# EduFdez/rgbd360

Hardware: AMD Instinct MI355X
Metric: Gauss-Newton iters/sec on 2048x1024 spherical pair; SE(3) err vs CPU ref (higher is better)
Workload: dtype f32; 1 GPU; configs[1]: single 2048x1024 synthetic sphere pair per GPU, PHOTO_CONSISTENCY RegisterPhotoICP, level-0 forced Gauss-Newton iterations (one launch each: solve of the previous pass + fused warp/residual/Jacobian pass); width=2048, height=1024, method=PHOTO_CONSISTENCY, n_pyr=4, pairs_per_gpu=1, parallelism=1 GPU

## Files before the change

rgbd360_amd/csrc/photo_icp_kernels.h:

```cpp
#pragma once
#include <hip/hip_runtime.h>
#include <stddef.h>
#include <stdint.h>

#include "device_math.h"
#include "gn_math.h"
#include "libm_f32.h"
#include "partial_row.h"

namespace r360 {

constexpr float  kInvalidPoint = -10000.f;
constexpr int    kEvalThreads = 1024;

struct F3 {
    float a, b, c;
};

struct LevelDev {
    int rows, cols, n;
    float half_nRows;
    float angle_res_inv;
    float pi_k;
    const float4* src;
// ... 530 lines not shown
    ESTAMP(4);
    if (threadIdx.x == 0 && (b == 0 || b == nb - 1)) {
        double* o = partials + (size_t)(nb + (b == 0 ? 0 : 1)) * kNumPartials;
        for (int k = 0; k < 5; ++k) o[k] = (double)es[k];
        o[5] = (double)es0;
        }
    if (threadIdx.x == 0) {
        double* pb = partials + (size_t)(nb + 8) * kNumPartials + 2 * b;
        pb[0] = (double)es0;
        pb[1] = (double)(es0 + es[4]);
    }
    if (threadIdx.x == 0 && b == 0) {
        {
            unsigned long long* cnt = reinterpret_cast<unsigned long long*>(partials + (size_t)(nb + 2) * kNumPartials);
            const unsigned long long slot = atomicAdd(cnt, 1ull) % 60;
            double* h = partials + (size_t)(nb + 3) * kNumPartials + 2 * slot;
            h[0] = (double)es0;
            h[1] = (double)(es0 + es[4]);
        }
    }
#endif
}

template <int METHOD, bool HG, int THREADS = kEvalThreads, int SRC = 0>
__device__ __forceinline__ void eval_block(const GNState* __restrict__ st, const float4* __restrict__ src0, const int n_px,
                                           const int chunk, const int level, const int nb_arg, double* __restrict__ partials,
                                           const LevelDev& lv, const EvalConsts& ec) {
    unsigned long long es[6] = {0, 0, 0, 0, 0, 0};
#ifdef RGBD360_EVAL_STAMPS
    const unsigned long long es0 = __builtin_amdgcn_s_memrealtime();
#else
    const unsigned long long es0 = 0;
#endif
    const int nb = nb_arg;
    const int b = blockIdx.x;
    const int cb = ((nb & 7) == 0) ? (b & 7) * (nb >> 3) + (b >> 3) : b;
    const int base = cb * chunk;
    const int end = min(base + chunk, n_px);
    EvalBufs bufs;
    bufs.src = make_rsrc(src0, (unsigned)n_px * 16u);
    bufs.trgP = make_rsrc(lv.trgP, (unsigned)lv.n * 12u);
    bufs.trgD = make_rsrc(lv.trgD, (unsigned)lv.n * 12u);
    bufs.row_bytes = (unsigned)lv.cols * 12u;
    const int i = base + (int)threadIdx.x;
    static_assert(THREADS == 1024 || THREADS == 512, "eval_block: 1024-lane layout, played by 1024 or 512 threads");
    SrcCursor cur = {0, 0, 0, 0};
    SrcForm<SRC>::cursor_init(cur, lv, i, THREADS);
    const typename SrcForm<SRC>::T sA = SrcForm<SRC>::load(lv, src0, n_px, base, (unsigned)threadIdx.x << 4, cur);
    const typename SrcForm<SRC>::T sB = SrcForm<SRC>::load(lv, src0, n_px, base + THREADS, (unsigned)threadIdx.x << 4, cur);
    const int2 gate = *reinterpret_cast<const int2*>(&st->done);
    const PoseRT T = load_pose(st->cand);
    const WarpConsts wc = make_warp_consts(T, lv);
    ESTAMP(0);
    PixW wA;
    warp_stage<METHOD, true, SRC>(sA, i < end, T, wc, lv, bufs, wA);
    asm volatile("" ::: "memory");
    if (gate.x | (gate.y != level)) return;
    ESTAMP(1);
    eval_span<METHOD, HG, THREADS, SRC>(T, wc, lv, ec, bufs, src0, n_px, base, end, b, nb, wA, sB, cur, partials, es, es0);
}

template <int METHOD, bool HG, int SRC = 0>
__global__ __launch_bounds__(kEvalThreads) void k_eval(const GNState* __restrict__ st, const float4* __restrict__ src0, int n_px,
                                                        int chunk, int level, int nb_arg, double* __restrict__ partials,
                                                        LevelDev lv, EvalConsts ec) {
    eval_block<METHOD, HG, kEvalThreads, SRC>(st, src0, n_px, chunk, level, nb_arg, partials, lv, ec);
}

constexpr int kEvalThreadsBatch = 512;
template <int METHOD, bool HG, int SRC = 0>
__global__ __launch_bounds__(kEvalThreadsBatch) void k_eval_b(const GNState* __restrict__ states, const float4* __restrict__ src0, int n_px,
                                                          int chunk, int level, int nb_arg, double* __restrict__ partials,
                                                          int partials_stride, LevelDev lv, EvalConsts ec) {
    const int slot = blockIdx.y;
    lv.trgP += (size_t)slot * (size_t)n_px;
    lv.trgD += (size_t)slot * (size_t)n_px;
    if (SRC == 2) lv.src2 += (size_t)slot * (size_t)n_px;
    eval_block<METHOD, HG, kEvalThreadsBatch, SRC>(states + slot, SRC == 0 ? src0 + (size_t)slot * (size_t)n_px : src0, n_px, chunk, level, nb_arg,
                                                   partials + (size_t)slot * (size_t)partials_stride, lv, ec);
}

struct PairTable {
    int trg[32], src[32];
};
template <int METHOD, bool HG, int SRC = 0>
__global__ __launch_bounds__(kEvalThreadsBatch) void k_eval_p(const GNState* __restrict__ states, const float4* __restrict__ src0, int n_px,
                                                          int chunk, int level, int nb_arg, double* __restrict__ partials,
                                                          int partials_stride, LevelDev lv, EvalConsts ec, PairTable pt) {
    const int slot = blockIdx.y;
    const size_t to = (size_t)pt.trg[slot] * (size_t)n_px, so = (size_t)pt.src[slot] * (size_t)n_px;
    lv.trgP += to;
    lv.trgD += to;
    if (SRC == 2) lv.src2 += so;
    eval_block<METHOD, HG, kEvalThreadsBatch, SRC>(states + slot, SRC == 0 ? src0 + so : src0, n_px, chunk, level, nb_arg,
                                                   partials + (size_t)slot * (size_t)partials_stride, lv, ec);
}

struct Pose16 {
    float v[16];
};
__device__ __forceinline__ void level_init_one(GNState* st, const Pose16& pose, int use_pose, int reset_all, int level);
struct FsInit {
    Pose16 pose;
    int on;
};
__global__ void k_level_init(GNState* st, Pose16 pose, int use_pose, int reset_all, int level) {
    if (threadIdx.x != 0 || blockIdx.x != 0) return;
    level_init_one(st, pose, use_pose, reset_all, level);
}
__global__ void k_level_init_b(GNState* states, Pose16 pose, int use_pose, int reset_all, int level, unsigned long long live_mask) {
    if (threadIdx.x != 0) return;
    GNState* st = states + blockIdx.x;
    if (!((live_mask >> blockIdx.x) & 1ull)) {
        st->done = 1;
        st->level_active = -1;
        st->status = 0;
        return;
    }
    level_init_one(st, pose, use_pose, reset_all, level);
}
__global__ void k_level_init_p(GNState* states, const Pose16* __restrict__ poses, int use_pose, int reset_all, int level,
                               unsigned long long live_mask) {
    if (threadIdx.x != 0) return;
    GNState* st = states + blockIdx.x;
    if (!((live_mask >> blockIdx.x) & 1ull)) {
        st->done = 1;
        st->level_active = -1;
        st->status = 0;
        return;
    }
    level_init_one(st, poses[blockIdx.x], use_pose, reset_all, level);
}
__device__ __forceinline__ void level_init_one(GNState* st, const Pose16& pose, int use_pose, int reset_all, int level) {
    if (reset_all) {
        for (int k = 0; k < 36; ++k) st->H[k] = st->Hused[k] = 0.f;
        for (int k = 0; k < 6; ++k) st->g[k] = st->gused[k] = 0.f;
        for (int k = 0; k < 8; ++k) st->iters[k] = 0;
        st->status = 0;
        st->n_evals = 0;
        st->acc_e2p = st->acc_e2d = 0.0;
        st->acc_np = st->acc_nd = st->acc_nvis = st->used_nvis = st->used_npix = 0;
    } else {
        if (st->status != 0 || !st->done || st->level_active != level + 1) return;
    }
    st->level_active = level;
    st->pend_nb = 0;
    if (use_pose)
        for (int k = 0; k < 16; ++k) st->pose[k] = pose.v[k];
    for (int k = 0; k < 16; ++k) st->cand[k] = st->pose[k];
    for (int k = 0; k < 6; ++k) st->update[k] = 1.f;
    st->lambda = 1.0;
    st->it = 0;
    st->first = 1;
    st->done = 0;
    st->error = st->new_error = st->diff_error = 0.0;
}

__device__ __forceinline__ float bcast(float v, int lane_uniform) {
    return __builtin_bit_cast(float, __builtin_amdgcn_readlane(__builtin_bit_cast(int, v), lane_uniform));
}

__device__ __forceinline__ bool lu_inverse6_lanes(const float* M , int lane, float x[6]) {
    float a[6];
#pragma unroll
    for (int r = 0; r < 6; ++r) a[r] = lane < 6 ? M[lane * 6 + r] : ((lane - 6) == r ? 1.f : 0.f);
    bool ok = true;
    float rk[6];
#pragma unroll
    for (int k = 0; k < 6; ++k) {
        float ck[6];
#pragma unroll
        for (int r = k; r < 6; ++r) ck[r] = bcast(a[r], k);
        int piv = k;
        unsigned best = __float_as_uint(ck[k]) & 0x7fffffffu;
#pragma unroll
        for (int r = k + 1; r < 6; ++r) {
            const unsigned v = __float_as_uint(ck[r]) & 0x7fffffffu;
            if (v > best) {
                best = v;
                piv = r;
            }
        }
        if (best == 0u) ok = false;
        const int pv = __builtin_amdgcn_readfirstlane(piv);
        if (pv != k) {
#pragma unroll
            for (int r = k + 1; r < 6; ++r)
                if (pv == r) {
                    asm volatile("v_swap_b32 %0, %1" : "+v"(a[k]), "+v"(a[r]));
                    const float t = ck[k]; ck[k] = ck[r]; ck[r] = t;
                }
        }
        rk[k] = rcp_rn(ck[k]);
#pragma unroll
        for (int r = k + 1; r < 6; ++r) {
            const float l = ck[r] * rk[k];
            if (lane > k) a[r] -= l * a[k];
        }
    }
#pragma unroll
    for (int r = 5; r >= 0; --r) {
        float sacc = a[r];
#pragma unroll
        for (int c = r + 1; c < 6; ++c) sacc -= bcast(a[r], c) * x[c];
        x[r] = sacc * rk[r];
    }
    return ok;
}

__device__ __forceinline__ int qr_rank6_lanes(const float* M , int lane) {
    const int col = lane < 6 ? lane : 5;
    float a[6];
#pragma unroll
    for (int r = 0; r < 6; ++r) a[r] = M[col * 6 + r];
    float sq = 0.f;
#pragma unroll
    for (int r = 0; r < 6; ++r) sq += a[r] * a[r];
    float maxColSq = 0.f;
#pragma unroll
    for (int c = 0; c < 6; ++c) {
        const float v = bcast(sq, c);
        maxColSq = v > maxColSq ? v : maxColSq;
    }
    const float threshold_helper = maxColSq * (gn::kEpsF * gn::kEpsF) / 6.f;
    float pivots[6] = {0.f, 0.f, 0.f, 0.f, 0.f, 0.f};
    float maxpivot = 0.f;
    int nonzero = 6;
    bool stopped = false;
#pragma unroll
    for (int k = 0; k < 6; ++k) {
        float sk = 0.f;
#pragma unroll
        for (int r = k; r < 6; ++r) sk += a[r] * a[r];
        int best = k;
        float bestSq = -1.f;
#pragma unroll
        for (int c = k; c < 6; ++c) {
            const float v = bcast(sk, c);
            if (v > bestSq) {
                bestSq = v;
                best = c;
            }
        }
        if (!stopped && bestSq < threshold_helper * (float)(6 - k)) {
            nonzero = k;
            stopped = true;
        }
        if (!stopped) {
            if (best != k) {
#pragma unroll
                for (int r = 0; r < 6; ++r) {
                    const float from_best = bcast(a[r], best), from_k = bcast(a[r], k);
                    a[r] = (lane == k) ? from_best : ((lane == best) ? from_k : a[r]);
                }
            }
            float ck[6];
#pragma unroll
            for (int r = 0; r < 6; ++r) ck[r] = bcast(a[r], k);
            float tailSq = 0.f;
#pragma unroll
            for (int r = k + 1; r < 6; ++r) tailSq += ck[r] * ck[r];
            const float c0 = ck[k];
            float beta, tau;
            float v[6] = {0.f, 0.f, 0.f, 0.f, 0.f, 0.f};
            if (tailSq == 0.f) {
                tau = 0.f;
                beta = c0;
            } else {
                beta = sqrtf(c0 * c0 + tailSq);
                if (c0 >= 0.f) beta = -beta;
                const float den = c0 - beta;
#pragma unroll
                for (int r = k + 1; r < 6; ++r) v[r] = ck[r] / den;
                tau = (beta - c0) / beta;
            }
            v[k] = 1.f;
            float dot = 0.f;
#pragma unroll
            for (int r = k; r < 6; ++r) dot += v[r] * a[r];
            dot *= tau;
            if (lane > k) {
#pragma unroll
                for (int r = k; r < 6; ++r) a[r] -= dot * v[r];
            }
            pivots[k] = beta;
            const float ab = fabsf(beta);
            maxpivot = ab > maxpivot ? ab : maxpivot;
        }
    }
    const float thr = maxpivot * (gn::kEpsF * 6.f);
    int rank = 0;
#pragma unroll
    for (int k = 0; k < 6; ++k) rank += (k < nonzero && fabsf(pivots[k]) > thr) ? 1 : 0;
    return rank;
}

constexpr int kSolveThreads = 1024;
struct SolveShared {
    GNState sst;
    double red[kSolveThreads / 64][kNumPartials];
    float shH[36], shM[36], shInv[36], shE[16], shCand[16], shUpd[6];
    int shGo, shRank, shLuOk;
    unsigned long long stamp0, stamp[8];
};
#ifdef RGBD360_SOLVE_STAMPS
#define SOLVE_STAMP_T(i, t) if (threadIdx.x == (t)) sh.stamp[i] = __builtin_amdgcn_s_memrealtime() - sh.stamp0
#else
#define SOLVE_STAMP_T(i, t)
#endif
#define SOLVE_STAMP(i) SOLVE_STAMP_T(i, 0)

__device__ __forceinline__ void reduce_rows_to_lds(SolveShared& sh, double s) {
    const double pair = add_other_half_d(s);
    if ((threadIdx.x & 63) < kNumPartials) sh.red[threadIdx.x >> 6][threadIdx.x & 31] = pair;
}
__device__ __forceinline__ float solve_totals(SolveShared& sh) {
    constexpr int Q = kSolveThreads / 64;
    const int tid = threadIdx.x;
    if (tid < kNumPartials) {
        double t = 0.0;
#pragma unroll
        for (int k = 0; k < Q; ++k) t += sh.red[k][tid];
        sh.sst.tot[tid] = t;
    }
    const float lam_spec = (float)(sh.sst.first ? sh.sst.lambda : sh.sst.lambda / 5.0);
    __syncthreads();
    SOLVE_STAMP_T(1, 0);
    return lam_spec;
}

__device__ __forceinline__ int solve_rank_wave(SolveShared& sh, const float lam_spec) {
    const int lane = threadIdx.x & 63;
    const double* tot = sh.sst.tot;
    float hval = 0.f;
    if (lane < 36) {
        const int r = lane / 6, c = lane - 6 * r;
        const int aa = r < c ? r : c, bb = r < c ? c : r;
        hval = (float)tot[P_H + (aa * (13 - aa)) / 2 + (bb - aa)];
        sh.shM[lane] = (lane % 7 == 0) ? hval + lam_spec * hval : hval;
    }
    const int rk = __builtin_amdgcn_readfirstlane(qr_rank6_lanes(sh.shM, lane));
    if (lane == 0) sh.shRank = rk;
    return rk;
}

__device__ __forceinline__ void solve_waves(SolveShared& sh, const SolveCfg& cfg, const float lam_spec, const bool rank_now) {
    const int tid = threadIdx.x, lane = tid & 63, wave = tid >> 6;
    GNState* st = &sh.sst;
    const double* tot = sh.sst.tot;
    if (cfg.mode == 0 && wave == 2 && rank_now) {
        solve_rank_wave(sh, lam_spec);
        SOLVE_STAMP_T(7, 128);
    }
    if (cfg.mode == 0 && wave == 1) {
        float hval = 0.f;
        if (lane < 36) {
            const int r = lane / 6, c = lane - 6 * r;
            const int aa = r < c ? r : c, bb = r < c ? c : r;
            hval = (float)tot[P_H + (aa * (13 - aa)) / 2 + (bb - aa)];
        }
        {
            if (lane < 36) sh.shH[lane] = hval;
            float x[6] = {0.f, 0.f, 0.f, 0.f, 0.f, 0.f};
            const bool ok = lu_inverse6_lanes(sh.shH, lane, x);
            if (lane >= 6 && lane < 12) {
#pragma unroll
                for (int r = 0; r < 6; ++r) sh.shInv[(lane - 6) * 6 + r] = x[r];
            }
            if (lane == 0) sh.shLuOk = ok ? 1 : 0;
            SOLVE_STAMP_T(5, 64);
            float upd = 0.f;
            if (lane < 6) {
#pragma unroll
                for (int c = 0; c < 6; ++c) upd += (-sh.shInv[c * 6 + lane]) * (float)tot[P_G + c];
                sh.shUpd[lane] = upd;
            }
            const double ux = (double)bcast(upd, 0), uy = (double)bcast(upd, 1), uz = (double)bcast(upd, 2);
            const double wx = (double)bcast(upd, 3), wy = (double)bcast(upd, 4), wz = (double)bcast(upd, 5);
            const double theta_sq = wx * wx + wy * wy + wz * wz;
            double ca = 0.0, cb = 0.0;
            const bool rot = theta_sq >= (128 * 2.220446049250313e-16) * (128 * 2.220446049250313e-16);
            if (rot) {
                if (theta_sq < 0.25) gn::sinc_cosc_sq(theta_sq, ca, cb);
                else gn::sinc_cosc(sqrt(theta_sq), ca, cb);
            }
            if (lane < 16) {
                const int i = lane & 3, j = lane >> 2;
                double e = (i == j) ? 1.0 : 0.0;
                if (i < 3 && j < 3) {
                    if (rot) {
                        const double wi = i == 0 ? wx : (i == 1 ? wy : wz), wj = j == 0 ? wx : (j == 1 ? wy : wz);
                        const int kk = 3 - i - j;
                        const double wk = kk == 0 ? wx : (kk == 1 ? wy : wz);
                        double Wij, W2ij;
                        if (i == j) {
                            Wij = 0.0;
                            const double first = i == 2 ? wy : wz, second = i == 0 ? wy : wx;
                            W2ij = (0.0 - first * first) - second * second;
                        } else {
                            Wij = ((j - i + 3) % 3 == 1) ? -wk : wk;
                            W2ij = wi * wj;
                        }
                        e += ca * Wij + cb * W2ij;
                    }
                } else if (j == 3 && i < 3) {
                    e = i == 0 ? ux : (i == 1 ? uy : uz);
                }
                sh.shE[lane] = (float)e;
            }
            if (lane < 16) {
                const int c = lane >> 2, r = lane & 3;
                const float* P = sh.sst.cand;
                sh.shCand[lane] = ((sh.shE[0 * 4 + r] * P[c * 4 + 0] + sh.shE[1 * 4 + r] * P[c * 4 + 1]) + sh.shE[2 * 4 + r] * P[c * 4 + 2]) +
                               sh.shE[3 * 4 + r] * P[c * 4 + 3];
            }
            SOLVE_STAMP_T(6, 64);
        }
    }
    if (wave == 0) {
        float hval = 0.f;
        if (lane < 36) {
            const int r = lane / 6, c = lane - 6 * r;
            const int aa = r < c ? r : c, bb = r < c ? c : r;
            hval = (float)tot[P_H + (aa * (13 - aa)) / 2 + (bb - aa)];
        } else if (lane < 42) {
            hval = (float)tot[P_G + lane - 36];
        }
        int take = 0, go = 0;
        if (lane == 0) {
            st->n_evals += 1;
            const double err2 = tot[P_E2P] + tot[P_E2D];
            const double nvalid = tot[P_NP] + tot[P_ND];
            const double new_error = cfg.occ == 0 ? sqrt(err2 / nvalid)
                                                  : sqrt(tot[P_E2P] / tot[P_NP]) + sqrt(tot[P_E2D] / tot[P_ND]);
            st->new_error = new_error;
            if (cfg.mode == 1) {
                take = 1;
            } else {
                bool stop = false;
                if (st->first) {
                    st->first = 0;
                    if (nvalid == 0.0 || new_error != new_error) {
                        st->status = 2;
                        st->done = 1;
                        stop = true;
                    } else {
                        st->error = new_error;
                        st->diff_error = new_error;
                        take = 1;
                    }
                } else {
                    const double diff = st->error - new_error;
                    st->diff_error = diff;
                    if (cfg.forced || diff > cfg.tol_residual) {
                        st->lambda = st->lambda / 5.0;
                        st->error = new_error;
                        st->it += 1;
                        st->iters[cfg.level & 7] = st->it;
                        take = 2;
                    }
                }
                if (take) {
                    st->acc_e2p = tot[P_E2P];
                    st->acc_e2d = tot[P_E2D];
                    st->acc_np = (long long)tot[P_NP];
                    st->acc_nd = (long long)tot[P_ND];
                    st->acc_nvis = (long long)tot[P_NVIS];
                }
                if (!stop) {
                    float un = 0.f;
                    for (int i = 0; i < 6; ++i) un += st->update[i] * st->update[i];
                    un = sqrtf(un);
                    go = cfg.forced || (st->it < cfg.max_iters && (double)un > cfg.tol_update && st->diff_error > cfg.tol_residual);
                    if (!go) st->done = 1;
                }
                if (go) {
                    st->used_nvis = st->acc_nvis;
                    st->used_npix = cfg.n_pixels;
                }
            }
            sh.shGo = go;
        }
        take = __builtin_amdgcn_readfirstlane(take);
        go = __builtin_amdgcn_readfirstlane(go);
        if (take == 2 && lane < 16) st->pose[lane] = st->cand[lane];
        if (take) {
            if (lane < 36) st->H[lane] = hval;
            else if (lane < 42) st->g[lane - 36] = hval;
        }
        if (go) {
            if (lane < 36) {
                st->Hused[lane] = hval;
            } else if (lane < 42) {
                st->gused[lane - 36] = hval;
            }
        }
    }
    SOLVE_STAMP(2);
}

__device__ __forceinline__ void solve_finish(SolveShared& sh, const SolveCfg& cfg) {
    const int tid = threadIdx.x;
    GNState* st = &sh.sst;
    if (sh.shGo) {
        const bool ill = (sh.shRank != 6) || !sh.shLuOk;
        if (ill) {
            if (tid == 0) {
                st->status = 1;
                st->done = 1;
            }
        } else if (tid < 16) {
            sh.sst.cand[tid] = sh.shCand[tid];
            if (tid < 6) sh.sst.update[tid] = sh.shUpd[tid];
        }
        SOLVE_STAMP(3);
        __syncthreads();
    }
    if (cfg.mode == 0 && !cfg.forced && cfg.level > 0 && sh.sst.done && sh.sst.status == 0) {
        __syncthreads();
        if (tid < 16) sh.sst.cand[tid] = sh.sst.pose[tid];
        if (tid < 6) sh.sst.update[tid] = 1.f;
        if (tid == 0) {
            sh.sst.level_active = cfg.level - 1;
            sh.sst.lambda = 1.0;
            sh.sst.it = 0;
            sh.sst.first = 1;
            sh.sst.done = 0;
            sh.sst.error = sh.sst.new_error = sh.sst.diff_error = 0.0;
        }
        __syncthreads();
    }
}

__device__ __forceinline__ void solve_staged(SolveShared& sh, const SolveCfg& cfg) {
    const float lam_spec = solve_totals(sh);
    solve_waves(sh, cfg, lam_spec, true);
    __syncthreads();
    solve_finish(sh, cfg);
}

__device__ __forceinline__ void solve_block(GNState* st_g, const double* __restrict__ partials, const int nb, const SolveCfg& cfg) {
    __shared__ SolveShared sh;
    constexpr int kStateWords = sizeof(GNState) / 4;
    static_assert(sizeof(GNState) % 4 == 0 && kStateWords <= kSolveThreads, "GNState staging");
    const int tid = threadIdx.x;
#ifdef RGBD360_SOLVE_STAMPS
    if (tid == 0) sh.stamp0 = __builtin_amdgcn_s_memrealtime();
#endif
    if (tid < kStateWords) reinterpret_cast<int*>(&sh.sst)[tid] = reinterpret_cast<const int*>(st_g)[tid];
    const int v = tid % kNumPartials, q = tid / kNumPartials;
    constexpr int Q = kSolveThreads / kNumPartials;
    double s = 0.0;
    for (int b0 = q; b0 < nb; b0 += 16 * Q) {
        double tmp[16];
#pragma unroll
        for (int j = 0; j < 16; ++j) {
            const int b = b0 + j * Q;
            tmp[j] = b < nb ? partials[(size_t)b * kNumPartials + v] : 0.0;
        }
#pragma unroll
        for (int j = 0; j < 16; ++j) s += tmp[j];
    }
    reduce_rows_to_lds(sh, s);
    __syncthreads();
    SOLVE_STAMP(0);
    if (cfg.mode == 0 && (sh.sst.done || sh.sst.level_active != cfg.level)) {
        if (cfg.host_state) {
            if (tid < 64) {
                for (int w = tid; w < kStateWords; w += 64) reinterpret_cast<int*>(cfg.host_state)[w] = reinterpret_cast<const int*>(&sh.sst)[w];
                __threadfence_system();
            }
            __syncthreads();
            if (tid == 0) __hip_atomic_store(cfg.host_tag, cfg.host_seq, __ATOMIC_RELEASE, __HIP_MEMORY_SCOPE_SYSTEM);
        }
        return;
    }
    solve_staged(sh, cfg);
#ifdef RGBD360_SOLVE_STAMPS
    if (tid == 0) {
        sh.stamp[4] = __builtin_amdgcn_s_memrealtime() - sh.stamp0;
        for (int i = 0; i < 8; ++i) sh.sst.stamps[i] = sh.stamp[i];
    }
    __syncthreads();
#endif
    if (tid < kStateWords) reinterpret_cast<int*>(st_g)[tid] = reinterpret_cast<const int*>(&sh.sst)[tid];
    if (cfg.host_state) {
        if (tid < 64) {
            for (int w = tid; w < kStateWords; w += 64) reinterpret_cast<int*>(cfg.host_state)[w] = reinterpret_cast<const int*>(&sh.sst)[w];
            __threadfence_system();
        }
        __syncthreads();
        if (tid == 0) __hip_atomic_store(cfg.host_tag, cfg.host_seq, __ATOMIC_RELEASE, __HIP_MEMORY_SCOPE_SYSTEM);
    }
}
__global__ __launch_bounds__(kSolveThreads) void k_solve(GNState* st_g, const double* __restrict__ partials, int nb,
                                                          SolveCfg cfg) {
    solve_block(st_g, partials, nb, cfg);
}
__global__ __launch_bounds__(kSolveThreads) void k_solve_b(GNState* states, const double* __restrict__ partials, int partials_stride,
                                                            int nb, SolveCfg cfg) {
    solve_block(states + blockIdx.x, partials + (size_t)blockIdx.x * (size_t)partials_stride, nb, cfg);
}

constexpr int kPendingRows = 256;
constexpr int kMaxPendingRows = kPendingRows;
__device__ __forceinline__ int stage_pending(SolveShared& sh, const GNState* __restrict__ st_in, const double* __restrict__ partials, const int rows_hint) {
    constexpr int kStateWords = sizeof(GNState) / 4;
    constexpr int Q = kSolveThreads / kNumPartials;
    constexpr int J = kPendingRows / Q;
    static_assert(J * Q == kPendingRows && J <= 16, "whole batches");
    const int tid = threadIdx.x;
    const int v = tid % kNumPartials, q = tid / kNumPartials;
    double tmp[J];
    tmp[0] = partials[(size_t)q * kNumPartials + v];
#pragma unroll
    for (int j = 1; j < J; ++j) tmp[j] = 0.0;
    if (rows_hint > Q) {
#pragma unroll
        for (int j = 1; j < J; ++j) tmp[j] = partials[(size_t)(q + j * Q) * kNumPartials + v];
    }
    int word = 0;
    if (tid < kStateWords) word = reinterpret_cast<const int*>(st_in)[tid];
    const int nb = st_in->pend_nb;
    if (nb > Q && rows_hint <= Q) {
#pragma unroll
        for (int j = 1; j < J; ++j) tmp[j] = partials[(size_t)(q + j * Q) * kNumPartials + v];
    }
#ifdef RGBD360_SOLVE_STAMPS
    if (tid == 0) sh.stamp[3] = __builtin_amdgcn_s_memrealtime();
#endif
    double s = 0.0;
#pragma unroll
    for (int j = 0; j < J; ++j) s += (q + j * Q < nb) ? tmp[j] : 0.0;
    reduce_rows_to_lds(sh, s);
    if (tid < kStateWords) reinterpret_cast<int*>(&sh.sst)[tid] = word;
#ifdef RGBD360_SOLVE_STAMPS
    if (tid == 0) {
        sh.stamp[5] = __builtin_amdgcn_s_memrealtime() - sh.stamp0;
        sh.stamp[3] -= sh.stamp0;
    }
#endif
    __syncthreads();
    return nb;
}

__device__ __forceinline__ float uniform_f(float v) {
    return __builtin_bit_cast(float, __builtin_amdgcn_readfirstlane(__builtin_bit_cast(int, v)));
}

struct FsDecision {
    bool run, commit, ill, handover;
    int level_now;
    float lam_spec;
};
__device__ __forceinline__ FsDecision fs_solve_decide(SolveShared& sh, const int pend, const SolveCfg& cfg, const int level, PoseRT& T) {
    float lam_spec = 0.f;
    int solved_level = 0;
    if (pend > 0) {
        SolveCfg c = cfg;
        c.level = solved_level = sh.sst.level_active;
        c.n_pixels = sh.sst.pend_npix;
        lam_spec = solve_totals(sh);
        solve_waves(sh, c, lam_spec, false);
        __syncthreads();
    }
    FsDecision d;
    const bool go = pend > 0 && sh.shGo != 0;
    d.commit = go && sh.shLuOk != 0;
    d.ill = go && !d.commit;
    d.handover = pend > 0 && !go && !cfg.forced && solved_level > 0 && sh.sst.done && sh.sst.status == 0;
    d.level_now = d.handover ? solved_level - 1 : sh.sst.level_active;
    const bool done_now = d.handover ? false : (d.ill || sh.sst.done != 0);
    d.run = !done_now && d.level_now == level;
    d.lam_spec = lam_spec;
    const float* P = d.commit ? sh.shCand : (d.handover ? sh.sst.pose : sh.sst.cand);
    T.r00 = uniform_f(P[0]); T.r10 = uniform_f(P[1]); T.r20 = uniform_f(P[2]);
    T.r01 = uniform_f(P[4]); T.r11 = uniform_f(P[5]); T.r21 = uniform_f(P[6]);
    T.r02 = uniform_f(P[8]); T.r12 = uniform_f(P[9]); T.r22 = uniform_f(P[10]);
    T.tx = uniform_f(P[12]); T.ty = uniform_f(P[13]); T.tz = uniform_f(P[14]);
    return d;
}
__device__ __forceinline__ void fs_write_state(SolveShared& sh, const FsDecision& d, const int nb, const int n_level_px, GNState* st_out) {
    constexpr int kStateWords = sizeof(GNState) / 4;
    const bool commit = d.commit, ill = d.ill, handover = d.handover, run = d.run;
    const int level_now = d.level_now;
    const int lane = threadIdx.x & 63;
    bool ill_late = false;
    if (commit) ill_late = solve_rank_wave(sh, d.lam_spec) != 6;
    const bool commit_f = commit && !ill_late, ill_f = ill || ill_late, run_f = run && !ill_late;
    constexpr int kCand = offsetof(GNState, cand) / 4, kUpd = offsetof(GNState, update) / 4;
    constexpr int kErr = offsetof(GNState, error) / 4, kLam = offsetof(GNState, lambda) / 4;
    static_assert(offsetof(GNState, new_error) == offsetof(GNState, error) + 8 && offsetof(GNState, diff_error) == offsetof(GNState, error) + 16, "error block");
    for (int w = lane; w < kStateWords; w += 64) {
        int val = reinterpret_cast<const int*>(&sh.sst)[w];
        if (w >= kCand && w < kCand + 16) {
            if (commit_f) val = __builtin_bit_cast(int, sh.shCand[w - kCand]);
            if (handover) val = __builtin_bit_cast(int, sh.sst.pose[w - kCand]);
        }
        if (w >= kUpd && w < kUpd + 6) {
            if (commit_f) val = __builtin_bit_cast(int, sh.shUpd[w - kUpd]);
            if (handover) val = __builtin_bit_cast(int, 1.f);
        }
        if (ill_f && (w == offsetof(GNState, status) / 4 || w == offsetof(GNState, done) / 4)) val = 1;
        if (handover) {
            if (w == offsetof(GNState, level_active) / 4) val = level_now;
            if (w == offsetof(GNState, it) / 4 || w == offsetof(GNState, done) / 4) val = 0;
            if (w == offsetof(GNState, first) / 4) val = 1;
            if (w >= kErr && w < kErr + 6) val = 0;
            if (w == kLam) val = 0;
            if (w == kLam + 1) val = 0x3FF00000;
        }
        if (w == offsetof(GNState, pend_nb) / 4) val = run_f ? nb : 0;
        if (w == offsetof(GNState, pend_npix) / 4) val = n_level_px;
#ifdef RGBD360_SOLVE_STAMPS
        if (w >= (int)offsetof(GNState, stamps) / 4 && w < (int)offsetof(GNState, stamps) / 4 + 16) {
            const int si = (w - (int)offsetof(GNState, stamps) / 4) >> 1;
            const unsigned long long sv = si == 4 ? __builtin_amdgcn_s_memrealtime() - sh.stamp0 : sh.stamp[si];
            val = (int)((w & 1) ? (sv >> 32) : (sv & 0xffffffffull));
        }
#endif
        reinterpret_cast<int*>(st_out)[w] = val;
    }
}
__device__ __forceinline__ bool fs_solve_and_publish(SolveShared& sh, const int pend, const SolveCfg& cfg, const int level, const int nb,
                                                     const int n_level_px, GNState* __restrict__ st_out, PoseRT& T) {
    const FsDecision d = fs_solve_decide(sh, pend, cfg, level, T);
    if (blockIdx.x == 0 && (threadIdx.x >> 6) == 2) fs_write_state(sh, d, nb, n_level_px, st_out);
    return d.run;
}

template <int METHOD, int SRC = 0>
__global__ __launch_bounds__(kEvalThreads) void k_eval_fs(const GNState* __restrict__ st_in, GNState* __restrict__ st_out,
                                                           const double* __restrict__ partials_in, double* __restrict__ partials_out,
                                                           const float4* __restrict__ src0, int n_px, int chunk, int level, int nb_arg,
                                                           int pend_rows_hint, LevelDev lv, EvalConsts ec, SolveCfg cfg, FsInit init) {
    static_assert(kEvalThreads == kSolveThreads, "the fused launch runs the solve on the pass's block");
    unsigned long long es[6] = {0, 0, 0, 0, 0, 0};
#ifdef RGBD360_EVAL_STAMPS
    const unsigned long long es0 = __builtin_amdgcn_s_memrealtime();
#else
    const unsigned long long es0 = 0;
#endif
    __shared__ SolveShared sh;
    constexpr int kStateWords = sizeof(GNState) / 4;
#ifdef RGBD360_SOLVE_STAMPS
    if (threadIdx.x == 0) sh.stamp0 = __builtin_amdgcn_s_memrealtime();
#endif
    int pend = stage_pending(sh, st_in, partials_in, pend_rows_hint);
    if (init.on) {
        if (threadIdx.x == 0) level_init_one(&sh.sst, init.pose, 1, 1, level);
        __syncthreads();
        pend = 0;
    }
    SOLVE_STAMP(0);
    const int nb = nb_arg;
    const int b = blockIdx.x;
    const int cb = ((nb & 7) == 0) ? (b & 7) * (nb >> 3) + (b >> 3) : b;
    const int base = cb * chunk;
    const int end = min(base + chunk, n_px);
    EvalBufs bufs;
    bufs.src = make_rsrc(src0, (unsigned)n_px * 16u);
    bufs.trgP = make_rsrc(lv.trgP, (unsigned)lv.n * 12u);
    bufs.trgD = make_rsrc(lv.trgD, (unsigned)lv.n * 12u);
    bufs.row_bytes = (unsigned)lv.cols * 12u;
    const int i = base + (int)threadIdx.x;
    SrcCursor cur = {0, 0, 0, 0};
    SrcForm<SRC>::cursor_init(cur, lv, i, kEvalThreads);
    const typename SrcForm<SRC>::T sA = SrcForm<SRC>::load(lv, src0, n_px, base, (unsigned)threadIdx.x << 4, cur);
    const typename SrcForm<SRC>::T sB = SrcForm<SRC>::load(lv, src0, n_px, base + kEvalThreads, (unsigned)threadIdx.x << 4, cur);
    PoseRT T;
    const bool run = fs_solve_and_publish(sh, pend, cfg, level, nb, lv.n, st_out, T);
    if (!run) return;
    const WarpConsts wc = make_warp_consts(T, lv);
    ESTAMP(0);
    PixW wA;
    warp_stage<METHOD, true, SRC>(sA, i < end, T, wc, lv, bufs, wA);
    ESTAMP(1);
    eval_span<METHOD, true, kEvalThreads, SRC>(T, wc, lv, ec, bufs, src0, n_px, base, end, b, nb, wA, sB, cur, partials_out, es, es0);
}

__global__ __launch_bounds__(kSolveThreads) void k_solve_pending(GNState* st_g, const double* __restrict__ partials, int pend_rows_hint,
                                                                  SolveCfg cfg) {
    __shared__ SolveShared sh;
    constexpr int kStateWords = sizeof(GNState) / 4;
    const int tid = threadIdx.x;
    const int pend = stage_pending(sh, st_g, partials, pend_rows_hint);
    if (pend > 0) {
        SolveCfg c = cfg;
        c.level = sh.sst.level_active;
        c.n_pixels = sh.sst.pend_npix;
        solve_staged(sh, c);
        if (tid == 0) sh.sst.pend_nb = 0;
        __syncthreads();
    }
    if (tid < kStateWords) reinterpret_cast<int*>(st_g)[tid] = reinterpret_cast<const int*>(&sh.sst)[tid];
    if (cfg.host_state) {
        if (tid < 64) {
            for (int w = tid; w < kStateWords; w += 64) reinterpret_cast<int*>(cfg.host_state)[w] = reinterpret_cast<const int*>(&sh.sst)[w];
            __threadfence_system();
        }
        __syncthreads();
        if (tid == 0) __hip_atomic_store(cfg.host_tag, cfg.host_seq, __ATOMIC_RELEASE, __HIP_MEMORY_SCOPE_SYSTEM);
    }
}

struct GnIO {
    float H[36], g[6], pose[16], pose_tmp[16], update[6];
    float lambda;
    int status;
};
__global__ void k_gn_step(GnIO* io) {
    if (threadIdx.x == 0 && blockIdx.x == 0) io->status = gn::step(io->H, io->g, io->lambda, io->pose, io->pose_tmp, io->update);
}

__global__ void k_warp_indices(LevelDev lv, Pose16 pose, int32_t* __restrict__ out) {
    const int i = blockIdx.x * blockDim.x + threadIdx.x;
    if (i >= lv.n) return;
    const PoseRT T = load_pose(pose.v);
    const float4 s = lv.src[i];
    int r = -1, c = -1;
    {
        float X, Y, Z, rho2, d2;
        bool vis;
        const WarpConsts wc = {T.tx, T.ty, T.tz, lv.half_nRows, lv.pi_k};
        const unsigned ti = warp_pixel(T, wc, s.x, s.y, s.z, lv, X, Y, Z, rho2, d2, vis);
        vis = vis && s.x != kInvalidPoint;
        if (vis) {
            r = (int)(ti / (unsigned)lv.cols);
            c = (int)ti - r * lv.cols;
        }
    }
    out[2 * i] = r;
    out[2 * i + 1] = c;
}

__global__ void k_selftest_math(unsigned first_bits, unsigned count, unsigned long long* __restrict__ mismatches) {
    const unsigned stride = gridDim.x * blockDim.x;
    unsigned bad_s = 0, bad_r = 0, bad_i = 0;
    if (blockIdx.x == 0 && threadIdx.x == 0) bad_s += (__builtin_bit_cast(unsigned, sqrt_rn(0.f)) != 0u);
    for (unsigned k = blockIdx.x * blockDim.x + threadIdx.x; k < count; k += stride) {
        const float x = __builtin_bit_cast(float, first_bits + k);
        const float s0 = sqrtf(x), s1 = sqrt_rn(x);
        const float r0 = 1.f / x, r1 = rcp_rn(x);
        const float q0 = 1.f / -x, q1 = rcp_rn(-x);
        bad_s += (__builtin_bit_cast(unsigned, s0) != __builtin_bit_cast(unsigned, s1));
        bad_r += (__builtin_bit_cast(unsigned, r0) != __builtin_bit_cast(unsigned, r1));
        bad_r += (__builtin_bit_cast(unsigned, q0) != __builtin_bit_cast(unsigned, q1));
        if (fabsf(x) < 1.0e9f) {
            bad_i += (round_index(x) != (int)floor((double)x + 0.5));
            bad_i += (round_index(-x) != (int)floor((double)(-x) + 0.5));
        }
    }
    if (bad_s) atomicAdd(&mismatches[0], (unsigned long long)bad_s);
    if (bad_r) atomicAdd(&mismatches[1], (unsigned long long)bad_r);
    if (bad_i) atomicAdd(&mismatches[2], (unsigned long long)bad_i);
}

__host__ __device__ __forceinline__ void selftest_libm_pair(unsigned k, float& y, float& x) {
    unsigned long long s = 0x9E3779B97F4A7C15ull * (k + 1ull);
    s ^= s << 13; s ^= s >> 7; s ^= s << 17;
    const unsigned long long r = s;
    s ^= s << 13; s ^= s >> 7; s ^= s << 17;
    const unsigned long long q = s;
    unsigned a = (unsigned)r, b = (unsigned)q;
    a = (a & 0x807fffffu) | ((87u + (unsigned)((r >> 32) % 81ull)) << 23);
    b = (b & 0x807fffffu) | ((87u + (unsigned)((q >> 32) % 81ull)) << 23);
    const unsigned kind = (unsigned)(r >> 40) & 63u;
    if (kind == 0) a &= 0x80000000u;
    if (kind == 1) b &= 0x80000000u;
    if (kind == 2) b = 0x3f800000u;
    if (kind == 3) b = (b & 0x80000000u) | (a & 0x7fffffffu);
    if (kind == 4) b = (b & 0x807fffffu) | (a & 0x7f800000u);
    y = libm32::u2f(a);
    x = libm32::u2f(b);
}
__global__ void k_selftest_libm(unsigned first_bits, unsigned count, float* __restrict__ out ) {
    const unsigned stride = gridDim.x * blockDim.x;
    for (unsigned k = blockIdx.x * blockDim.x + threadIdx.x; k < count; k += stride) {
        const float v = libm32::u2f(first_bits + k);
        out[k] = libm32::asinf_(v);
        out[(size_t)count + k] = libm32::atanf_(v);
        out[2 * (size_t)count + k] = libm32::roundf_(v);
        float y, x;
        selftest_libm_pair(first_bits + k, y, x);
        out[3 * (size_t)count + k] = libm32::atan2f_(y, x);
    }
}

__device__ __forceinline__ void gray_u8_x4(const uint8_t* __restrict__ rgb, size_t step, int rows, int cols, float* __restrict__ out,
                                           int c4, int r) {
    if (c4 >= cols || r >= rows) return;
    const uint8_t* p = rgb + (size_t)r * step + 3 * (size_t)c4;
    float* o = out + (size_t)r * cols + c4;
    const float k = (float)(1. / 255);
    auto gray = [](unsigned a, unsigned b, unsigned c) { return (int)((4899u * a + 9617u * b + 1868u * c + 8192u) >> 14); };
    if (c4 + 4 <= cols && (((size_t)p | (size_t)o) & 3) == 0 && ((size_t)o & 15) == 0) {
        const uint32_t* q = reinterpret_cast<const uint32_t*>(p);
        const uint32_t w0 = q[0], w1 = q[1], w2 = q[2];
        float4 v;
        v.x = (float)gray(w0 & 255u, (w0 >> 8) & 255u, (w0 >> 16) & 255u) * k;
        v.y = (float)gray(w0 >> 24, w1 & 255u, (w1 >> 8) & 255u) * k;
        v.z = (float)gray((w1 >> 16) & 255u, w1 >> 24, w2 & 255u) * k;
        v.w = (float)gray((w2 >> 8) & 255u, (w2 >> 16) & 255u, w2 >> 24) * k;
        *reinterpret_cast<float4*>(o) = v;
    } else {
        for (int j = 0; j < 4 && c4 + j < cols; ++j) o[j] = (float)gray(p[3 * j], p[3 * j + 1], p[3 * j + 2]) * k;
    }
}

__device__ __forceinline__ void depth_to_f32_x4(const void* __restrict__ depth, size_t step, int depth_type, int rows, int cols,
                                                float* __restrict__ out, int c4, int r) {
    if (c4 >= cols || r >= rows) return;
    const uint8_t* row = (const uint8_t*)depth + (size_t)r * step;
    float* o = out + (size_t)r * cols + c4;
    if (depth_type == 0) {
        const uint16_t* p = (const uint16_t*)row + c4;
        if (c4 + 4 <= cols && ((size_t)p & 7) == 0 && ((size_t)o & 15) == 0) {
            const uint2 w = *reinterpret_cast<const uint2*>(p);
            *reinterpret_cast<float4*>(o) = make_float4((float)(w.x & 0xFFFFu) * 0.001f, (float)(w.x >> 16) * 0.001f,
                                                        (float)(w.y & 0xFFFFu) * 0.001f, (float)(w.y >> 16) * 0.001f);
        } else {
            for (int j = 0; j < 4 && c4 + j < cols; ++j) o[j] = (float)p[j] * 0.001f;
        }
    } else {
        const float* p = (const float*)row + c4;
        for (int j = 0; j < 4 && c4 + j < cols; ++j) o[j] = p[j];
    }
}

__global__ void k_convert_pair(const uint8_t* __restrict__ rgb, size_t rgb_step, const void* __restrict__ depth, size_t depth_step,
                               int depth_type, int rows, int cols, float* __restrict__ gray_out, float* __restrict__ depth_out) {
    const int c4 = (blockIdx.x * blockDim.x + threadIdx.x) * 4;
    const int r = blockIdx.y;
    if (blockIdx.z == 0) gray_u8_x4(rgb, rgb_step, rows, cols, gray_out, c4, r);
    else depth_to_f32_x4(depth, depth_step, depth_type, rows, cols, depth_out, c4, r);
}

__device__ __forceinline__ int reflect101(int i, int n) {
    if (n == 1) return 0;
    while (i < 0 || i >= n) i = (i < 0) ? -i : 2 * n - 2 - i;
    return i;
}

__device__ __forceinline__ void pyrdown_gray_px(const float* __restrict__ src, int srows, int scols, float* __restrict__ dst,
                                                int dcols, int x, int y) {
    int cc[5], rr[5];
#pragma unroll
    for (int k = 0; k < 5; ++k) {
        cc[k] = reflect101(2 * x - 2 + k, scols);
        rr[k] = reflect101(2 * y - 2 + k, srows);
    }
    float h[5];
#pragma unroll
    for (int k = 0; k < 5; ++k) {
        const float* row = src + (size_t)rr[k] * scols;
        h[k] = row[cc[2]] * 6 + (row[cc[1]] + row[cc[3]]) * 4 + row[cc[0]] + row[cc[4]];
    }
    const float v = h[2] * 6 + (h[1] + h[3]) * 4 + h[0] + h[4];
    dst[(size_t)y * dcols + x] = v * (1.f / 256.f);
}

__device__ __forceinline__ void pyrdown_depth_px(const float* __restrict__ src, int scols, float* __restrict__ dst, int dcols,
                                                 float min_depth, float max_depth, int x, int y) {
    float av = 0.f;
    unsigned n = 0;
#pragma unroll
    for (int i = 0; i < 2; ++i)
#pragma unroll
        for (int j = 0; j < 2; ++j) {
            const float z = src[(size_t)(2 * y + i) * scols + 2 * x + j];
            if (z > min_depth && z < max_depth) {
                av += z;
                ++n;
            }
        }
    dst[(size_t)y * dcols + x] = n > 0 ? av / n : 0.f;
}

__global__ void k_pyrdown_pair(const float* __restrict__ gray_src, const float* __restrict__ depth_src, int srows, int scols,
                               float* __restrict__ gray_dst, float* __restrict__ depth_dst, int drows, int dcols, float min_depth,
                               float max_depth) {
    const int x = blockIdx.x * blockDim.x + threadIdx.x;
    const int y = blockIdx.y;
    if (x >= dcols || y >= drows) return;
    if (blockIdx.z == 0) pyrdown_gray_px(gray_src, srows, scols, gray_dst, dcols, x, y);
    else pyrdown_depth_px(depth_src, scols, depth_dst, dcols, min_depth, max_depth, x, y);
}

__device__ __forceinline__ void gradient_rec_px(const float* __restrict__ src, int rows, int cols, int seam_width,
                                                F3* __restrict__ rec, int r, int c) {
    const float v = src[(size_t)r * cols + c];
    float gx = 0.f, gy = 0.f;
    if (r >= 1 && r < rows - 1 && c >= 1 && c < cols - 1) {
        const float xm = src[(size_t)r * cols + c - 1], xp = src[(size_t)r * cols + c + 1];
        const float ym = src[(size_t)(r - 1) * cols + c], yp = src[(size_t)(r + 1) * cols + c];
        if ((v > xp && v < xm) || (v < xp && v > xm)) gx = 2.f / (1 / (xp - v) + 1 / (v - xm));
        if ((v > yp && v < ym) || (v < yp && v > ym)) gy = 2.f / (1 / (yp - v) + 1 / (v - ym));
    }
    if (seam_width > 1) {
        int s, rem;
        divmod24(c + 1, seam_width, s, rem);
        if (rem <= 1 && s >= 1 && s <= 7) gx = gy = 0.f;
    } else if (seam_width == 1) {
        if (c + 1 >= 1 && c <= 7) gx = gy = 0.f;
    }
    F3 o;
    o.a = v; o.b = gx; o.c = gy;
    rec[(size_t)r * cols + c] = o;
}

constexpr int kMaxJobs = 16;
struct GradJobs {
    const float* src[kMaxJobs];
    F3*          rec[kMaxJobs];
    int rows[kMaxJobs], cols[kMaxJobs], seam[kMaxJobs], first_block[kMaxJobs + 1];
    int n;
};
__global__ void k_gradient_rec_multi(GradJobs jobs) {
    int j = 0;
    while (j + 1 < jobs.n && (int)blockIdx.x >= jobs.first_block[j + 1]) ++j;
    const int p = ((int)blockIdx.x - jobs.first_block[j]) * (int)blockDim.x + (int)threadIdx.x;
    const int cols = jobs.cols[j], rows = jobs.rows[j];
    if (p >= rows * cols) return;
    int r, c;
    divmod24(p, cols, r, c);
    gradient_rec_px(jobs.src[j], rows, cols, jobs.seam[j], jobs.rec[j], r, c);
}

__device__ __forceinline__ void src_rec_px(const float* __restrict__ depth, const float* __restrict__ gray, int cols,
                                           const float* __restrict__ sin_theta, const float* __restrict__ cos_theta,
                                           const float* __restrict__ sin_phi, const float* __restrict__ cos_phi, float min_depth,
                                           float max_depth, float4* __restrict__ rec, int r, int c) {
    const size_t i = (size_t)r * cols + c;
    const float d = depth[i];
    float4 o;
    o.w = gray[i];
    if (min_depth < d && d < max_depth) {
        o.x = d * sin_phi[r];
        o.y = -d * cos_phi[r] * sin_theta[c];
        o.z = -d * cos_phi[r] * cos_theta[c];
    } else {
        o.x = kInvalidPoint;
        o.y = 0.f;
        o.z = 0.f;
    }
    rec[i] = o;
}
struct SrcJobs {
    const float *depth[8], *gray[8], *sin_theta[8], *cos_theta[8], *sin_phi[8], *cos_phi[8];
    float4* rec[8];
    int rows[8], cols[8], first_block[9];
    int n;
    float min_depth, max_depth;
};
__global__ void k_src_rec_multi(SrcJobs jobs) {
    int j = 0;
    while (j + 1 < jobs.n && (int)blockIdx.x >= jobs.first_block[j + 1]) ++j;
    const int p = ((int)blockIdx.x - jobs.first_block[j]) * (int)blockDim.x + (int)threadIdx.x;
    const int cols = jobs.cols[j], rows = jobs.rows[j];
    if (p >= rows * cols) return;
    int r, c;
    divmod24(p, cols, r, c);
    src_rec_px(jobs.depth[j], jobs.gray[j], cols, jobs.sin_theta[j], jobs.cos_theta[j], jobs.sin_phi[j], jobs.cos_phi[j],
               jobs.min_depth, jobs.max_depth, jobs.rec[j], r, c);
}

constexpr int kMaxSlots = 32;
struct FramePtrs {
    const uint8_t* rgb[kMaxSlots];
    const void* depth[kMaxSlots];
};
__global__ void k_convert_pair_b(FramePtrs fp, size_t rgb_step, size_t depth_step, int depth_type, int rows, int cols,
                                 float* __restrict__ gray_out, float* __restrict__ depth_out, unsigned long long live_mask) {
    const int slot = blockIdx.z >> 1;
    if (!((live_mask >> slot) & 1ull)) return;
    const int c4 = (blockIdx.x * blockDim.x + threadIdx.x) * 4;
    const int r = blockIdx.y;
    const size_t off = (size_t)slot * (size_t)rows * (size_t)cols;
    if ((blockIdx.z & 1) == 0) gray_u8_x4(fp.rgb[slot], rgb_step, rows, cols, gray_out + off, c4, r);
    else depth_to_f32_x4(fp.depth[slot], depth_step, depth_type, rows, cols, depth_out + off, c4, r);
}
__global__ void k_pyrdown_pair_b(const float* __restrict__ gray_src, const float* __restrict__ depth_src, int srows, int scols,
                                 float* __restrict__ gray_dst, float* __restrict__ depth_dst, int drows, int dcols, float min_depth,
                                 float max_depth, unsigned long long live_mask) {
    const int slot = blockIdx.z >> 1;
    if (!((live_mask >> slot) & 1ull)) return;
    const int x = blockIdx.x * blockDim.x + threadIdx.x;
    const int y = blockIdx.y;
    if (x >= dcols || y >= drows) return;
    const size_t so = (size_t)slot * (size_t)srows * (size_t)scols, dof = (size_t)slot * (size_t)drows * (size_t)dcols;
    if ((blockIdx.z & 1) == 0) pyrdown_gray_px(gray_src + so, srows, scols, gray_dst + dof, dcols, x, y);
    else pyrdown_depth_px(depth_src + so, scols, depth_dst + dof, dcols, min_depth, max_depth, x, y);
}
__global__ void k_gradient_rec_multi_b(GradJobs jobs, unsigned long long live_mask) {
// ... 280 lines not shown
```

Baseline: 68430 GN iterations/s.

## Fuse 6x6 LU inverse, update, and exp-map into one wavefront solve path

Adds a fast-track solve path that runs the Hessian load, the 6x6 LU inverse, the Gauss-Newton update, the SE(3) exponential and the candidate pose multiply inside a single wavefront using lane broadcasts and branchless selects. Pose and Hessian bookkeeping runs concurrently in wave 0, and the rank check runs in wave 2. The aim is to shorten the serial tail of the solve, which sits on the critical path of every launch, by cutting barriers and divergent per-stage work. The LU first tries elimination without pivot swaps and falls back to a pivoting pass when a swap is needed, which adds branches and code size. An optional compile-time dry-run mode, used for timing, is also added.

```diff
diff --git a/rgbd360_amd/csrc/photo_icp_kernels.h b/rgbd360_amd/csrc/photo_icp_kernels.h
--- a/rgbd360_amd/csrc/photo_icp_kernels.h
+++ b/rgbd360_amd/csrc/photo_icp_kernels.h
@@ -856,6 +856,10 @@
     float shH[36], shM[36], shInv[36], shE[16], shCand[16], shUpd[6];
     int shGo, shRank, shLuOk;
     unsigned long long stamp0, stamp[8];
+#ifdef RGBD360_SOLVE_TWICE
+    float dry[36 + 36 + 16 + 16 + 6];
+    int dryLuOk;
+#endif
 };
 #ifdef RGBD360_SOLVE_STAMPS
 #define SOLVE_STAMP_T(i, t) if (threadIdx.x == (t)) sh.stamp[i] = __builtin_amdgcn_s_memrealtime() - sh.stamp0
@@ -1092,7 +1096,6 @@
     __syncthreads();
     solve_finish(sh, cfg);
 }
-
 __device__ __forceinline__ void solve_block(GNState* st_g, const double* __restrict__ partials, const int nb, const SolveCfg& cfg) {
     __shared__ SolveShared sh;
     constexpr int kStateWords = sizeof(GNState) / 4;
@@ -1198,6 +1201,260 @@
     return nb;
 }
 
+__device__ __forceinline__ void solve_bookkeeping_wave(SolveShared& sh, const SolveCfg& cfg, const int lane) {
+    GNState* st = &sh.sst;
+    const double* tot = sh.sst.tot;
+    float hval = 0.f;
+    if (lane < 36) {
+        const int r = lane / 6, c = lane - 6 * r;
+        const int aa = r < c ? r : c, bb = r < c ? c : r;
+        hval = (float)tot[P_H + (aa * (13 - aa)) / 2 + (bb - aa)];
+    } else if (lane < 42) {
+        hval = (float)tot[P_G + lane - 36];
+    }
+    int take = 0, go = 0;
+    if (lane == 0) {
+        st->n_evals += 1;
+        const double err2 = tot[P_E2P] + tot[P_E2D];
+        const double nvalid = tot[P_NP] + tot[P_ND];
+        const double new_error = cfg.occ == 0 ? sqrt(err2 / nvalid)
+                                              : sqrt(tot[P_E2P] / tot[P_NP]) + sqrt(tot[P_E2D] / tot[P_ND]);
+        st->new_error = new_error;
+        if (cfg.mode == 1) {
+            take = 1;
+        } else {
+            bool stop = false;
+            if (st->first) {
+                st->first = 0;
+                if (nvalid == 0.0 || new_error != new_error) {
+                    st->status = 2;
+                    st->done = 1;
+                    stop = true;
+                } else {
+                    st->error = new_error;
+                    st->diff_error = new_error;
+                    take = 1;
+                }
+            } else {
+                const double diff = st->error - new_error;
+                st->diff_error = diff;
+                if (cfg.forced || diff > cfg.tol_residual) {
+                    st->lambda = st->lambda / 5.0;
+                    st->error = new_error;
+                    st->it += 1;
+                    st->iters[cfg.level & 7] = st->it;
+                    take = 2;
+                }
+            }
+            if (take) {
+                st->acc_e2p = tot[P_E2P];
+                st->acc_e2d = tot[P_E2D];
+                st->acc_np = (long long)tot[P_NP];
+                st->acc_nd = (long long)tot[P_ND];
+                st->acc_nvis = (long long)tot[P_NVIS];
+            }
+            if (!stop) {
+                float un = 0.f;
+                for (int i = 0; i < 6; ++i) un += st->update[i] * st->update[i];
+                un = sqrtf(un);
+                go = cfg.forced || (st->it < cfg.max_iters && (double)un > cfg.tol_update && st->diff_error > cfg.tol_residual);
+                if (!go) st->done = 1;
+            }
+            if (go) {
+                st->used_nvis = st->acc_nvis;
+                st->used_npix = cfg.n_pixels;
+            }
+        }
+        sh.shGo = go;
+    }
+    take = __builtin_amdgcn_readfirstlane(take);
+    go = __builtin_amdgcn_readfirstlane(go);
+    if (take == 2 && lane < 16) st->pose[lane] = st->cand[lane];
+    if (take) {
+        if (lane < 36) st->H[lane] = hval;
+        else if (lane < 42) st->g[lane - 36] = hval;
+    }
+    if (go) {
+        if (lane < 36) {
+            st->Hused[lane] = hval;
+        } else if (lane < 42) {
+            st->gused[lane - 36] = hval;
+        }
+    }
+}
+
+struct SolveWave1Slots {
+    float *H, *Inv, *E, *Cand, *Upd;
+    int* LuOk;
+};
+__device__ __forceinline__ int solve_h_slot(const int lane) {
+    const int l = lane < 36 ? lane : 35;
+    const int r = l / 6, c = l - 6 * r;
+    const int aa = r < c ? r : c, bb = r < c ? c : r;
+    return P_H + (aa * (13 - aa)) / 2 + (bb - aa);
+}
+__device__ __forceinline__ void lu_load6_ft(const float* M, const int lane, float a[6]) {
+    const bool is_m = lane < 6;
+    const int col = is_m ? lane : 5;
+#pragma unroll
+    for (int r = 0; r < 6; ++r) {
+        const float m = M[col * 6 + r];
+        const float id = (lane - 6) == r ? 1.f : 0.f;
+        a[r] = is_m ? m : id;
+    }
+}
+template <bool SWAPS>
+__device__ __forceinline__ bool lu_eliminate6_ft(float a[6], float rk[6], const int lane, bool& ok) {
+    bool in_place = true;
+#pragma unroll
+    for (int k = 0; k < 6; ++k) {
+        float ck[6];
+#pragma unroll
+        for (int r = k; r < 6; ++r) ck[r] = bcast(a[r], k);
+        int piv = k;
+        unsigned best = __float_as_uint(ck[k]) & 0x7fffffffu;
+#pragma unroll
+        for (int r = k + 1; r < 6; ++r) {
+            const unsigned v = __float_as_uint(ck[r]) & 0x7fffffffu;
+            if (v > best) {
+                best = v;
+                piv = r;
+            }
+        }
+        ok = best == 0u ? false : ok;
+        if (SWAPS) {
+            const int pv = __builtin_amdgcn_readfirstlane(piv);
+            if (pv != k) {
+#pragma unroll
+                for (int r = k + 1; r < 6; ++r)
+                    if (pv == r) {
+                        asm volatile("v_swap_b32 %0, %1" : "+v"(a[k]), "+v"(a[r]));
+                        const float t = ck[k]; ck[k] = ck[r]; ck[r] = t;
+                    }
+            }
+        } else {
+            in_place = piv != k ? false : in_place;
+        }
+        rk[k] = rcp_rn(ck[k]);
+        const bool below = lane > k;
+#pragma unroll
+        for (int r = k + 1; r < 6; ++r) {
+            const float l = ck[r] * rk[k];
+            const float t = a[r] - l * a[k];
+            a[r] = below ? t : a[r];
+        }
+    }
+    return in_place;
+}
+__device__ __forceinline__ bool lu_inverse6_lanes_ft(const float* M , int lane, float x[6]) {
+    float a[6], rk[6];
+    bool ok = true;
+    lu_load6_ft(M, lane, a);
+    if (__builtin_expect(!lu_eliminate6_ft<false>(a, rk, lane, ok), 0)) {
+        ok = true;
+        lu_load6_ft(M, lane, a);
+        lu_eliminate6_ft<true>(a, rk, lane, ok);
+    }
+#pragma unroll
+    for (int r = 5; r >= 0; --r) {
+        float sacc = a[r];
+#pragma unroll
+        for (int c = r + 1; c < 6; ++c) sacc -= bcast(a[r], c) * x[c];
+        x[r] = sacc * rk[r];
+    }
+    return ok;
+}
+template <typename T>
+__device__ __forceinline__ T pick(const bool c, const T a, const T b) {
+    return c ? a : b;
+}
+__device__ __forceinline__ void solve_exp_coeffs_rare(const double theta_sq, const bool rot, double& ca, double& cb) {
+    ca = 0.0;
+    cb = 0.0;
+    if (rot) gn::sinc_cosc(sqrt(theta_sq), ca, cb);
+}
+__device__ __forceinline__ void solve_wave1_ft(SolveShared& sh, const SolveWave1Slots& o, const int lane, const int h_slot,
+                                               const int stamp_inv, const int stamp_cand) {
+    const double* tot = sh.sst.tot;
+    const int l36 = lane < 36 ? lane : 35, l16 = lane & 15, l6 = lane < 6 ? lane : 5;
+    o.H[l36] = (float)tot[h_slot];
+    float x[6] = {0.f, 0.f, 0.f, 0.f, 0.f, 0.f};
+    const bool ok = lu_inverse6_lanes_ft(o.H, lane, x);
+#pragma unroll
+    for (int r = 0; r < 6; ++r) asm volatile("" : "+v"(x[r]));
+    float* const own = o.Inv + (lane - 6) * 6;
+    __shared__ float nobodys_slots[36];
+    float* const nobodys = nobodys_slots + l6 * 6;
+    float* const xcol = pick(lane >= 6 && lane < 12, own, nobodys);
+#pragma unroll
+    for (int r = 0; r < 6; ++r) xcol[r] = x[r];
+    *o.LuOk = ok ? 1 : 0;
+    SOLVE_STAMP_T(stamp_inv, 64);
+    float upd = 0.f;
+#pragma unroll
+    for (int c = 0; c < 6; ++c) upd += (-o.Inv[c * 6 + l6]) * (float)tot[P_G + c];
+    o.Upd[l6] = upd;
+    const double ux = (double)bcast(upd, 0), uy = (double)bcast(upd, 1), uz = (double)bcast(upd, 2);
+    const double wx = (double)bcast(upd, 3), wy = (double)bcast(upd, 4), wz = (double)bcast(upd, 5);
+    const double theta_sq = wx * wx + wy * wy + wz * wz;
+    double ca, cb;
+    const bool rot = theta_sq >= (128 * 2.220446049250313e-16) * (128 * 2.220446049250313e-16);
+    if (__builtin_expect(rot && theta_sq < 0.25, 1)) gn::sinc_cosc_sq(theta_sq, ca, cb);
+    else solve_exp_coeffs_rare(theta_sq, rot, ca, cb);
+    {
+        const int i = l16 & 3, j = l16 >> 2, kk = 3 - i - j;
+        const bool on_diag = i == j, rot_part = i < 3 && j < 3, trans_part = j == 3 && i < 3, minus = (j - i + 3) % 3 == 1;
+        const double diag = pick(on_diag, 1.0, 0.0);
+        const double wi = pick(i == 0, wx, pick(i == 1, wy, wz)), wj = pick(j == 0, wx, pick(j == 1, wy, wz));
+        const double wk = pick(kk == 0, wx, pick(kk == 1, wy, wz));
+        const double first = pick(i == 2, wy, wz), second = pick(i == 0, wy, wx);
+        double W2d = (0.0 - first * first) - second * second, W2o = wi * wj;
+        asm volatile("" : "+v"(W2d), "+v"(W2o));
+        const double Wij = pick(on_diag, 0.0, pick(minus, -wk, wk));
+        const double W2ij = pick(on_diag, W2d, W2o);
+        double er = diag + (ca * Wij + cb * W2ij);
+        asm volatile("" : "+v"(er));
+        const double ut = pick(i == 0, ux, pick(i == 1, uy, uz));
+        const double e = pick(rot_part, pick(rot, er, diag), pick(trans_part, ut, diag));
+        o.E[l16] = (float)e;
+    }
+    {
+        const int c = l16 >> 2, r = l16 & 3;
+        const float* P = sh.sst.cand;
+        o.Cand[l16] = ((o.E[0 * 4 + r] * P[c * 4 + 0] + o.E[1 * 4 + r] * P[c * 4 + 1]) + o.E[2 * 4 + r] * P[c * 4 + 2]) + o.E[3 * 4 + r] * P[c * 4 + 3];
+    }
+    SOLVE_STAMP_T(stamp_cand, 64);
+}
+__device__ __forceinline__ void solve_waves_ft(SolveShared& sh, const SolveCfg& cfg, const float lam_spec, const bool rank_now, const int h_slot) {
+    const int lane = threadIdx.x & 63;
+    const int wave = __builtin_amdgcn_readfirstlane((int)(threadIdx.x >> 6));
+    if (__builtin_expect(cfg.mode == 0 && wave == 1, 1)) {
+#ifdef RGBD360_SOLVE_TWICE
+        const SolveWave1Slots dry = {sh.dry, sh.dry + 36, sh.dry + 72, sh.dry + 88, sh.dry + 104, &sh.dryLuOk};
+        solve_wave1_ft(sh, dry, lane, h_slot, 7, 2);
+#endif
+        const SolveWave1Slots out = {sh.shH, sh.shInv, sh.shE, sh.shCand, sh.shUpd, &sh.shLuOk};
+        solve_wave1_ft(sh, out, lane, h_slot, 5, 6);
+    } else if (wave == 0) {
+        solve_bookkeeping_wave(sh, cfg, lane);
+    } else if (cfg.mode == 0 && wave == 2 && rank_now) {
+        solve_rank_wave(sh, lam_spec);
+        SOLVE_STAMP_T(7, 128);
+    }
+#ifndef RGBD360_SOLVE_TWICE
+    SOLVE_STAMP(2);
+#endif
+}
+
+__device__ __forceinline__ void solve_staged_ft(SolveShared& sh, const SolveCfg& cfg) {
+    int h_slot = solve_h_slot(threadIdx.x & 63);
+    asm volatile("" : "+v"(h_slot));
+    const float lam_spec = solve_totals(sh);
+    solve_waves_ft(sh, cfg, lam_spec, true, h_slot);
+    __syncthreads();
+    solve_finish(sh, cfg);
+}
+
 __device__ __forceinline__ float uniform_f(float v) {
     return __builtin_bit_cast(float, __builtin_amdgcn_readfirstlane(__builtin_bit_cast(int, v)));
 }
@@ -1214,8 +1471,10 @@
         SolveCfg c = cfg;
         c.level = solved_level = sh.sst.level_active;
         c.n_pixels = sh.sst.pend_npix;
+        int h_slot = solve_h_slot(threadIdx.x & 63);
+        asm volatile("" : "+v"(h_slot));
         lam_spec = solve_totals(sh);
-        solve_waves(sh, c, lam_spec, false);
+        solve_waves_ft(sh, c, lam_spec, false, h_slot);
         __syncthreads();
     }
     FsDecision d;
@@ -1343,7 +1602,7 @@
         SolveCfg c = cfg;
         c.level = sh.sst.level_active;
         c.n_pixels = sh.sst.pend_npix;
-        solve_staged(sh, c);
+        solve_staged_ft(sh, c);
         if (tid == 0) sh.sst.pend_nb = 0;
         __syncthreads();
     }
```

Measured after the change: 70550 GN iterations/s, median of 6. 1.03x the previous value.
